# pityka/lamp

Hardware: AMD Instinct MI355X
Metric: training-step samples/sec (higher is better)
Workload: dtype bf16; 1 GPU; example-cifar100 Cnn.resnet(100) training step (fwd+backprop+AdamW), synthetic CIFAR batch; per_gpu_batch=2048, global_batch=2048, parallelism=single, optimizer=AdamW lr 1e-3 wd 0 beta2 0.95 mixedPrecision

## Files before the change

lamp_amd/csrc/core/switches.h:

```cpp
#pragma once
#include <cstdint>

namespace lamp {

constexpr int64_t SW_NO_CLAMP = INT64_MIN;

#define LAMP_SWITCHES_ONCE(X)                                                                                                             \
                                                        \
  X(conv_sibling, "LAMP_CONV_SIBLING", BOOL, 1, 0, "a residual block's 3x3 and its sibling 1x1 of the same input as one forward launch") \
  X(conv_chain, "LAMP_CONV_CHAIN", BOOL, 1, 0, "a convolution directly in front of a residual block and the block's 3x3 + 1x1 as one forward call (0: two)") \
  X(fuse_bn_pair, "LAMP_FUSE_BN_PAIR", BOOL, 1, 0, "relu(bn(right) + bn(left)) at a block's end as one op (0: the chain)")                \
  X(fuse_pool_logsoftmax, "LAMP_FUSE_POOL_LOGSOFTMAX", BOOL, 1, 0, "average pool -> flatten -> log-softmax tail as one node")             \
  X(fuse_block_tail, "LAMP_FUSE_BLOCK_TAIL", BOOL, 1, 0, "the last residual block and the pooled log-softmax tail as one node")          \
  X(fuse_bn_conv, "LAMP_FUSE_BN_CONV", BOOL, 1, 0, "batch norm -> relu -> convolution: the convolution applies the norm while staging")  \
  X(fuse_loss_accumulate, "LAMP_FUSE_LOSS_ACCUMULATE", BOOL, 1, 0, "acc += n * loss inside the NLL loss kernel")                          \
  X(fuse_loss_backward, "LAMP_FUSE_LOSS_BACKWARD", BOOL, 1, 0, "the NLL loss backward goes straight to the pooled log-softmax node's input in one launch")                      \
  X(fuse_loss_tail, "LAMP_FUSE_LOSS_TAIL", BOOL, 1, 0, "the loss launch also writes the pooled log-softmax's input gradient per plane")  \
  X(conv_dgrad_accumulate, "LAMP_CONV_DGRAD_ACCUMULATE", BOOL, 1, 0, "a convolution's input gradient adds into the existing one in its epilogue") \
  X(conv_dgrad_pair, "LAMP_CONV_DGRAD_PAIR", BOOL, 1, 0, "input gradients of a block's 3x3 and sibling 1x1 from one launch")             \
  X(conv_wgrad_pair, "LAMP_CONV_WGRAD_PAIR", BOOL, 1, 0, "weight gradients of a block's 3x3 and sibling 1x1 from one launch")            \
  X(conv_bwd_pair, "LAMP_CONV_BWD_PAIR", BOOL, 1, 0, "a block's paired input gradient and its two weight gradients from one call (0: the two pair calls)") \
  X(linear_bias_fused, "LAMP_LINEAR_BIAS_FUSED", BOOL, 1, 0, "a linear layer's bias in the GEMM epilogue (0: mm then add)")               \
  X(mult_add_fused, "LAMP_MULT_ADD_FUSED", BOOL, 1, 0, "x * scale + residual in one pass (0: mult then add)")                             \
  X(attention_as_written_for_cuda, "LAMP_ATTENTION_AS_WRITTEN_FOR_CUDA", BOOL, 0, 0, "multi-head attention as the reference's op chain instead of the fused kernels") \
  X(recurrent_fused, "LAMP_RECURRENT_FUSED", BOOL, 1, 0, "RNN / GRU / LSTM as one node per sequence with fused cell kernels (0: the fold over time steps)") \
  X(fuse_qkv, "LAMP_FUSE_QKV", BOOL, 1, 0, "self-attention's three projections as one product (0: three)")                                \
  X(host_stream_side, "LAMP_HOST_STREAM_SIDE", BOOL, 0, 0, "batch streams gather on a side stream instead of the consumer's")             \
                                                                           \
  X(pinned_cache_mb, "LAMP_PINNED_CACHE_MB", INT, 2048, 0, "upper bound of the cache of freed pinned host buffers, MiB")                  \
  X(pinned_gather_wgs, "LAMP_PINNED_GATHER_WGS", INT, 48, 1, "workgroups of a gather that reads pinned host memory")                      \
                                                                                                    \
  X(flash_attention, "LAMP_FLASH_ATTENTION", BOOL, 1, 0, "the flash attention kernels, forward and backward")                             \
  X(small_attention, "LAMP_SMALL_ATTENTION", BOOL, 1, 0, "the short-sequence attention kernels")                                          \
  X(knn_fused, "LAMP_KNN_FUSED", BOOL, 1, 0, "the fused distance + top-k nearest-neighbour kernel")                                       \
  X(knn_split, "LAMP_KNN_SPLIT", INT, -1, SW_NO_CLAMP, "f16-plane k-NN filter: 0 off, 1 where it pays, 2 forced; negative: the mode set through the API") \
  X(knn_split_planes, "LAMP_KNN_SPLIT_PLANES", INT, 0, SW_NO_CLAMP, "f16 planes per coordinate of that filter: 3, anything else 2")      \
  X(umap_pairs2, "LAMP_UMAP_PAIRS2", BOOL, 1, 0, "the UMAP loss's two-dimensional pair kernel")                                            \
                                                                                                             \
  X(gemm_shape_tags, "LAMP_GEMM_SHAPE_TAGS", BOOL, 0, 0, "profiling aid: one kernel-timer class per GEMM shape and layout")               \
  X(gemm_splitk, "LAMP_GEMM_SPLITK", BOOL, 1, 0, "split-K for products with few output tiles (bf16 and f32 / f64)")                       \
  X(gemm_tail_split, "LAMP_GEMM_TAIL_SPLIT", BOOL, 1, 0, "an almost empty last round of 256 x 256 tiles becomes a second, split-K product") \
  X(gemm_fp_split_wgs, "LAMP_GEMM_FP_SPLIT_WGS", INT, 512, 1, "workgroups an f32 / f64 split-K product aims at")                          \
                                                                                              \
  X(bn_fused_bwd, "LAMP_BN_FUSED_BWD", BOOL, 1, 0, "one-pass batch-norm backward (workgroups exchange their sums) where no mode is set through the API") \
  X(bn_fused_fp, "LAMP_BN_FUSED_FP", BOOL, 1, 0, "... its f32 / f64 form")                                                               \
  X(bn_fused_np_mask, "LAMP_BN_FUSED_NP_MASK", INT, 24, SW_NO_CLAMP, "bit mask of packets per thread (1 .. 16) at which the one-pass form runs") \
  X(bn_fused_per_cu, "LAMP_BN_FUSED_PER_CU", INT, 1, 1, "workgroups per CU the one-pass form aims at first")                              \
  X(bn_fused_small_bytes, "LAMP_BN_FUSED_SMALL_BYTES", INT, (4 << 20) + 1, SW_NO_CLAMP, "bf16 activations below this many bytes take the one-pass form whatever the mask") \
                          \
  X(conv_small2, "LAMP_CONV_SMALL2", BOOL, 1, 0, "the small-map direct convolution kernels (second generation)")                          \
  X(conv_small2_wgrad, "LAMP_CONV_SMALL2_WGRAD", BOOL, 1, 0, "... their weight gradient")                                                 \
  X(igemm_f32, "LAMP_IGEMM_F32", BOOL, 1, 0, "implicit-GEMM convolution for f32")                                                          \
  X(igemm_f64, "LAMP_IGEMM_F64", BOOL, 1, 0, "implicit-GEMM convolution for f64")                                                          \
  X(conv_bn_stats, "LAMP_CONV_BN_STATS", BOOL, 1, 0, "forward convolutions hand per-image batch-norm statistics of their output on")     \
  X(ncv_bn_stats, "LAMP_NCV_BN_STATS", BOOL, 1, 0, "... the narrow kernels' alone (needs LAMP_CONV_BN_STATS on as well)")                 \
  X(ncv_dgrad_parity, "LAMP_NCV_DGRAD_PARITY", BOOL, 1, 0, "narrow stride-2 pair input gradient: super-tiles by row parity (0: the plain form)") \
  X(pack_cache, "LAMP_PACK_CACHE", BOOL, 1, 0, "packed filter images are cached per parameter and storage version (all four packing backends: core/pack_cache.h)") \
  X(pack_after_step, "LAMP_PACK_AFTER_STEP", BOOL, 1, 0, "the optimiser repacks every cached filter image of all four backends in place (0: lazily at first use)") \
                                                    \
  X(ig_small_d, "LAMP_IG_SMALL_D", BOOL, 1, 0, "the eight-image kernel for at most 64 output channels too")                               \
  X(ig_w8, "LAMP_IG_W8", BOOL, 1, 0, "two-image 128-row kernel: eight waves per image pair at one workgroup per CU or fewer (0: four)")  \
  X(ig_one_image, "LAMP_IG_ONE_IMAGE", BOOL, 1, 0, "... one image per workgroup at one image per CU or fewer (0: pairs)")                 \
  X(ig_bwd_pair, "LAMP_IG_BWD_PAIR", BOOL, 1, 0, "a wide block's short-K entry pair: input gradient and both weight gradients from one eight-image launch (0: the two pair calls)") \
  X(ig_fwd_pair, "LAMP_IG_FWD_PAIR", BOOL, 1, 0, "a wide block's short-K entry pair, forward: the barrier-free eight-image kernel with both filters resident in LDS (0: the eight-image kernel's sibling form)") \
                                                                                                 \
  X(wgrad_group, "LAMP_WGRAD_GROUP", BOOL, 1, 0, "two layers' eight-wave weight gradients parked and launched as one (0: every layer at once)") \
  X(wgrad_min_ips, "LAMP_WGRAD_MIN_IPS", INT, 0, 2, "fewest images per weight-gradient workgroup; unset (0): 2 up to 512 images, 8 above") \
  X(wg8h_dma, "LAMP_WG8H_DMA", BOOL, 1, 0, "eight-wave weight-gradient kernel: dY tiles by LDS-DMA (0: through registers, the bitwise reference of the DMA's hand-counted waits)") \
  X(defer_wgrad_reduce, "LAMP_DEFER_WGRAD_REDUCE", BOOL, 1, 0, "weight-gradient partial sums are reduced in batches, deferred until someone reads them")

#define LAMP_SWITCHES_PER_CALL(X)                                                                                                         \
  X(ig_variant, "LAMP_IG_VARIANT", LETTER, 0, 0, "bf16 implicit GEMM kernel form: b two-image 128-row, d eight-image at any batch; unset or any other letter: by geometry") \
  X(ig_ktail, "LAMP_IG_KTAIL", BOOL, 1, 0, "a 3x3's 1 .. 8 channels beyond the last whole K chunk from their own packed image (0: the padded chunk)") \
  X(knn_split_dbg, "LAMP_KNN_SPLIT_DBG", INT, 0, SW_NO_CLAMP, "3: the k-NN filter's kernel counts visits, candidates and selection cycles per wave and prints them")

using SwType_BOOL = bool;
using SwType_INT = int64_t;
using SwType_LETTER = char;
#define LAMP_SWITCH_MEMBER(member, name, kind, dflt, lo, doc) SwType_##kind member;
struct Switches { LAMP_SWITCHES_ONCE(LAMP_SWITCH_MEMBER) };
struct SwitchesNow { LAMP_SWITCHES_PER_CALL(LAMP_SWITCH_MEMBER) };
#undef LAMP_SWITCH_MEMBER

const Switches& sw();
SwitchesNow sw_now();

}
```

lamp_amd/csrc/host/ops.cpp:

```cpp
#include "ops.h"
#include "../core/switches.h"
#include <cstring>
#include <map>
#include <tuple>

#include <unordered_set>

namespace lamp {
namespace host {

Var make_const(const Ten& t) {
  auto v = std::make_shared<Variable>();
  v->value = t;
  return v;
}
Var make_param(const Ten& t) {
  auto v = std::make_shared<Variable>();
  v->value = t;
  v->wants_grad = true;
  return v;
}
Var make_result(const std::shared_ptr<Op>& op, const Ten& value) {
  auto v = std::make_shared<Variable>();
  v->op = op;
// ... 632 lines not shown
        cache->p = p;
      }
      acc.accumulate(cache->g[which], true);
      cache->g[which] = Ten();
      if (!cache->g[0].defined() && !cache->g[1].defined() && !cache->g[2].defined()) cache->p = Ten();
    };
  };
  op->params.push_back({query, back(0)});
  op->params.push_back({key, back(1)});
  op->params.push_back({value, back(2)});
  return make_result(op, out);
}

struct ConvPairGrad {
  struct Side { Ten w; std::vector<int64_t> stride, padding, dilation; Ten p; Ten pw; Variable* wout = nullptr; };
  Side side[2];
  int64_t groups = 1;
  int waiting = -1;
  int wwaiting = -1;
  Ten dw[2], dwp;
  void drop_merged() { dw[0] = Ten(); dw[1] = Ten(); dwp = Ten(); }
};
static Var convolution_node(const Var& input, const Var& weight, const Var& bias, const std::vector<int64_t>& stride,
                            const std::vector<int64_t>& padding, const std::vector<int64_t>& dilation, bool transposed,
                            const std::vector<int64_t>& outputPadding, int64_t groups, const Ten* computed,
                            const std::shared_ptr<ConvPairGrad>& pair = nullptr, int pair_side = 0) {
  auto op = new_op("Convolution");
  const int ns = (int)stride.size();
  Ten iv = input->value, wv = weight->value;
  const bool fuse_accumulate = sw().conv_dgrad_accumulate;
  const bool fuse_pair = sw().conv_dgrad_pair;
  const bool fuse_bwd_pair = sw().conv_bwd_pair && sw().conv_wgrad_pair;
  Variable* const wvar = weight.get();
  auto back = [=](int which) {
    std::function<void(const Ten&, Variable&)> single;
    single = [=](const Ten& p, Variable& out) {
      if (which == 0 && !transposed && fuse_accumulate && out.has_grad() && out.grad.h()->is_device() && p.h()->is_device() && out.grad.dtype() == p.dtype()) {
        lamp_tensor* r = nullptr;
        HCALL(lamp_convolution_backward_input_add(&r, p.h(), iv.h(), wv.h(), stride.data(), padding.data(), dilation.data(), ns,
                                                  outputPadding.data(), groups, out.grad.h()));
        out.grad = Ten(r);
        out.grad_shared = false;
        return;
      }
      lamp_tensor* o3[3] = {nullptr, nullptr, nullptr};
      uint8_t mask[3] = {(uint8_t)(which == 0), (uint8_t)(which == 1), (uint8_t)(which == 2)};
      HCALL(lamp_convolution_backward(o3, p.h(), iv.h(), wv.h(), stride.data(), padding.data(), dilation.data(), ns, transposed,
                                      outputPadding.data(), groups, mask));
      out.accumulate(Ten(o3[which]), true);
    };
    const bool fuse_wpair = sw().conv_wgrad_pair;
    if (which == 1 && pair && fuse_wpair && !transposed) {
      Variable* inp = input.get();
      return Backward([=](const Ten& p, Variable& out) {
        if (!p.h()->is_device() || tls_backprop_hooked || out.op) { single(p, out); return; }
        ConvPairGrad& st = *pair;
        if (st.wwaiting < 0) {
          st.wwaiting = pair_side;
          st.side[pair_side].pw = p;
          st.side[pair_side].wout = &out;
          inp->pending.push_back([=] {
            ConvPairGrad& s2 = *pair;
            if (s2.wwaiting != pair_side) return;
            s2.drop_merged();
            const Ten held = s2.side[pair_side].pw;
            Variable* wo = s2.side[pair_side].wout;
            s2.side[pair_side].pw = Ten(); s2.side[pair_side].wout = nullptr; s2.wwaiting = -1;
            single(held, *wo);
          });
          return;
        }
        if (st.wwaiting == pair_side) { single(p, out); return; }
        const int other = st.wwaiting;
        const Ten po = st.side[other].pw;
        Variable* wo = st.side[other].wout;
        st.side[other].pw = Ten(); st.side[other].wout = nullptr; st.wwaiting = -1;
        if (st.dw[0].defined() && st.dwp.defined() && st.dwp.h() == p.h()) {
          const Ten da = st.dw[0], db = st.dw[1];
          st.drop_merged();
          (pair_side == 0 ? out : *wo).accumulate(da, true);
          (pair_side == 0 ? *wo : out).accumulate(db, true);
// ... 28 lines not shown
        });
        return;
      }
      if (st.waiting == pair_side) { single(p, out); return; }
      const int other = st.waiting;
      const Ten po = st.side[other].p;
      st.side[other].p = Ten(); st.waiting = -1;
      const Ten& pa = pair_side == 0 ? p : po;
      const Ten& pb = pair_side == 0 ? po : p;
      const bool have = out.has_grad() && out.grad.h()->is_device() && out.grad.dtype() == p.dtype();
      if (out.has_grad() && !have) { single(po, out); single(p, out); return; }
      if (fuse_bwd_pair && !tls_backprop_hooked && st.wwaiting == other && st.side[other].pw.defined() && st.side[other].pw.h() == po.h() &&
          st.side[other].wout && !wvar->op && wvar->needsGrad() && wvar->value.h()->is_device()) {
        lamp_tensor* o3[3] = {nullptr, nullptr, nullptr};
        HCALL(lamp_convolution_backward_pair(o3, iv.h(), pa.h(), st.side[0].w.h(), st.side[0].stride.data(), st.side[0].padding.data(),
                                             st.side[0].dilation.data(), pb.h(), st.side[1].w.h(), st.side[1].stride.data(),
                                             st.side[1].padding.data(), st.side[1].dilation.data(), ns, st.groups, have ? out.grad.h() : nullptr));
        out.grad = Ten(o3[0]);
        out.grad_shared = false;
        st.dw[0] = Ten(o3[1]); st.dw[1] = Ten(o3[2]); st.dwp = p;
        return;
      }
      lamp_tensor* r = nullptr;
      HCALL(lamp_convolution_backward_input_pair(&r, iv.h(), pa.h(), st.side[0].w.h(), st.side[0].stride.data(), st.side[0].padding.data(),
                                                 st.side[0].dilation.data(), pb.h(), st.side[1].w.h(), st.side[1].stride.data(),
                                                 st.side[1].padding.data(), st.side[1].dilation.data(), ns, st.groups, have ? out.grad.h() : nullptr));
      out.grad = Ten(r);
      out.grad_shared = false;
    });
  };
  op->params.push_back({input, back(0)});
  op->params.push_back({weight, back(1)});
  op->params.push_back({bias, back(2)});
  if (pair) op->reset = [pair] {
    pair->waiting = pair->wwaiting = -1;
    for (auto& sd : pair->side) { sd.p = Ten(); sd.pw = Ten(); sd.wout = nullptr; }
    pair->drop_merged();
  };
  if (computed) return make_result(op, *computed);
  lamp_tensor* o = nullptr;
  HCALL(lamp_convolution(&o, iv.h(), wv.h(), bias->value.h(), stride.data(), padding.data(), dilation.data(), ns, transposed,
                         outputPadding.data(), groups));
  return make_result(op, Ten(o));
}
Var convolution(const Var& input, const Var& weight, const Var& bias, const std::vector<int64_t>& stride,
                const std::vector<int64_t>& padding, const std::vector<int64_t>& dilation, bool transposed,
                const std::vector<int64_t>& outputPadding, int64_t groups) {
  return convolution_node(input, weight, bias, stride, padding, dilation, transposed, outputPadding, groups, nullptr);
}
static std::pair<Var, Var> convolution_pair_nodes(const Var& input, const Var& weight_a, const Var& bias_a, const std::vector<int64_t>& stride_a,
                                                  const std::vector<int64_t>& padding_a, const std::vector<int64_t>& dilation_a, const Var& weight_b,
                                                  const Var& bias_b, const std::vector<int64_t>& stride_b, const std::vector<int64_t>& padding_b,
                                                  const std::vector<int64_t>& dilation_b, int64_t groups, const Ten& ya, const Ten& yb);
std::pair<Var, Var> convolution_pair(const Var& input, const Var& weight_a, const Var& bias_a, const std::vector<int64_t>& stride_a,
                                     const std::vector<int64_t>& padding_a, const std::vector<int64_t>& dilation_a, const Var& weight_b,
                                     const Var& bias_b, const std::vector<int64_t>& stride_b, const std::vector<int64_t>& padding_b,
                                     const std::vector<int64_t>& dilation_b, int64_t groups) {
  const int ns = (int)stride_a.size();
  LAMP_CHECK(ns == (int)stride_b.size(), "convolution_pair: the two convolutions have different numbers of spatial dimensions");
  lamp_tensor* o2[2] = {nullptr, nullptr};
  HCALL(lamp_convolution_pair(o2, input->value.h(), weight_a->value.h(), bias_a->value.h(), stride_a.data(), padding_a.data(), dilation_a.data(),
                              weight_b->value.h(), bias_b->value.h(), stride_b.data(), padding_b.data(), dilation_b.data(), ns, groups));
  return convolution_pair_nodes(input, weight_a, bias_a, stride_a, padding_a, dilation_a, weight_b, bias_b, stride_b, padding_b, dilation_b, groups, Ten(o2[0]),
                                Ten(o2[1]));
}
static std::pair<Var, Var> convolution_pair_nodes(const Var& input, const Var& weight_a, const Var& bias_a, const std::vector<int64_t>& stride_a,
// ... 419 lines not shown
```

lamp_amd/csrc/kernels/conv.hip:

```cpp
#include "device_utils.h"
#include "../core/strided.h"
#include "../core/switches.h"
#include "conv_geom.h"
#include "conv_backends.h"

namespace lamp {

template <class T>
__global__ __launch_bounds__(256) void conv_fwd_direct_kernel(const T* __restrict__ x, const T* __restrict__ w, const T* __restrict__ bias,
                                                              T* __restrict__ y, ConvGeom g) {
  using A = acc_t<T>;
  const int64_t total = g.N * g.Cout * g.Ho * g.Wo;
  const int cin_g = (int)(g.Cin / g.groups), cout_g = (int)(g.Cout / g.groups);
  for (int64_t e = blockIdx.x * (int64_t)blockDim.x + threadIdx.x; e < total; e += (int64_t)gridDim.x * blockDim.x) {
    const int wo = (int)(e % g.Wo);
    const int ho = (int)((e / g.Wo) % g.Ho);
    const int co = (int)((e / (g.Wo * g.Ho)) % g.Cout);
    const int64_t n = e / (g.Wo * g.Ho * g.Cout);
    const int grp = co / cout_g;
    A acc = bias ? load_as<A>(bias[co]) : A(0);
    const T* wp = w + (int64_t)co * cin_g * g.kh * g.kw;
    for (int cl = 0; cl < cin_g; cl++) {
      const T* xp = x + ((n * g.Cin + grp * cin_g + cl) * g.H) * g.W;
      for (int r = 0; r < g.kh; r++) {
// ... 373 lines not shown
      }
    }
  }
  if (!fused) {
    lamp_tensor* s = nullptr;
    if (lamp_convolution(&s, x, w, bias, stride, padding, dilation, nspatial, 0, zero2, groups) != 0) throw Error(lamp_last_error());
    Hold hs(s);
    lamp_tensor* o2[2] = {nullptr, nullptr};
    if (lamp_convolution_pair(o2, s, w_a, bias_a, stride_a, padding_a, dilation_a, w_b, bias_b, stride_b, padding_b, dilation_b, nspatial, groups) != 0)
      throw Error(lamp_last_error());
    out3[0] = hs.take(); out3[1] = o2[0]; out3[2] = o2[1];
  }
  LAMP_API_END
}

int lamp_convolution_backward(lamp_tensor* out3[3], const lamp_tensor* grad_out, const lamp_tensor* x, const lamp_tensor* w,
                              const int64_t* stride, const int64_t* padding, const int64_t* dilation, int nspatial, int transposed,
                              const int64_t* output_padding, int64_t groups, const uint8_t mask[3]) {
  LAMP_API_BEGIN
  check_device_tensor(x, "input"); check_device_tensor(w, "weight"); check_device_tensor(grad_out, "grad_out");
  LAMP_CHECK(x->dtype == w->dtype && grad_out->dtype == x->dtype, "convolution_backward: dtype mismatch");
  ConvGeom g = make_geom(x, w, stride, padding, dilation, nspatial, transposed, output_padding, groups);
  {
    const int64_t oc = transposed ? g.Cin : g.Cout, oh = transposed ? g.H : g.Ho, ow = transposed ? g.W : g.Wo;
    LAMP_CHECK(grad_out->ndim == x->ndim && grad_out->sizes[0] == g.N && grad_out->sizes[1] == oc &&
               grad_out->sizes[grad_out->ndim - 1] == ow && (nspatial == 1 || grad_out->sizes[2] == oh),
               "convolution_backward: grad_out " << grad_out->describe() << " does not match the forward output shape");
  }
  Hold xc(contiguous(x)), wc(contiguous_filter(w)), gc(contiguous(grad_out));
  hipStream_t st = current_stream(x->device());
  Hold dx(mask[0] ? new_like(xc.get()) : nullptr);
  Hold dw(mask[1] ? new_like(wc.get()) : nullptr);
  Hold db;
  if (!transposed) {
    if (dx.get() && !igemm_conv_dgrad(gc.get(), wc.get(), dx.get(), g, st) && !igemm32_conv_dgrad(gc.get(), wc.get(), dx.get(), g, st) &&
        !narrow_conv_dgrad(gc.get(), wc.get(), dx.get(), g, st) && !small_conv_dgrad(gc.get(), wc.get(), dx.get(), g, st)) {
      LAMP_DISPATCH_FLOAT(x->dtype, T, (launch_dgrad<T>(gc.get(), wc.get(), nullptr, dx.get(), g, st)));
    }
    if (dw.get() && !igemm_conv_wgrad(gc.get(), xc.get(), dw.get(), g, st) && !igemm32_conv_wgrad(gc.get(), xc.get(), dw.get(), g, st) &&
        !narrow_conv_wgrad(gc.get(), xc.get(), dw.get(), g, st) && !small_conv_wgrad(gc.get(), xc.get(), dw.get(), g, st)) {
      LAMP_DISPATCH_FLOAT(x->dtype, T, (launch_wgrad<T>(gc.get(), xc.get(), dw.get(), g, st)));
    }
  } else {
    if (dx.get()) { LAMP_DISPATCH_FLOAT(x->dtype, T, (launch_fwd<T>(gc.get(), wc.get(), nullptr, dx.get(), g, st))); }
    if (dw.get()) { LAMP_DISPATCH_FLOAT(x->dtype, T, (launch_wgrad<T>(xc.get(), gc.get(), dw.get(), g, st))); }
  }
  if (mask[2]) {
    std::vector<int64_t> dims = {0};
    for (int i = 2; i < grad_out->ndim; i++) dims.push_back(i);
    db = Hold(reduce_dims(gc.get(), dims.data(), (int)dims.size(), false, 0));
  }
  out3[0] = dx.take(); out3[1] = dw.take(); out3[2] = db.take();
  LAMP_API_END
}

static void check_affine(const lamp_tensor* affine, const lamp_tensor* x) {
  check_device_tensor(affine, "affine");
  LAMP_CHECK(affine->dtype == kF32 && affine->ndim == 2 && affine->sizes[0] == x->sizes[1] && affine->sizes[1] == 4 && affine->is_contiguous(),
             "affine must be the contiguous f32 [channels, 4] table of lamp_batch_norm_affine, got " << affine->describe());
  LAMP_CHECK(x->dtype == kBF16 || x->dtype == kF16 || x->dtype == kF32, "conv(relu(bn(x))) with a folded batch norm is a reduced-precision path (f32 table): f64 runs the separate operators");
}
int lamp_convolution_bn_relu_input_folds(int* out, const lamp_tensor* x, const lamp_tensor* w, const int64_t* stride, const int64_t* padding,
                                         const int64_t* dilation, int nspatial, int64_t groups) {
  LAMP_API_BEGIN
  *out = 0;
  if (!x->is_device() || !w->is_device() || x->dtype != w->dtype) return 0;
  const int64_t zero2[2] = {0, 0};
// ... 220 lines not shown
```

lamp_amd/csrc/kernels/conv_backends.h:

```cpp
#pragma once
#include "../core/tensor.h"
#include "conv_geom.h"

namespace lamp {
struct NcvPackMany;

bool igemm_conv_fwd(const Tensor* x, const Tensor* w, const Tensor* bias, Tensor* y, const ConvGeom& g, hipStream_t st);
bool igemm_conv_fwd_pair(const Tensor* x, const Tensor* w, const Tensor* bias, Tensor* y, const ConvGeom& g, const Tensor* w1, const Tensor* bias1,
                         Tensor* y1, const ConvGeom& g1, hipStream_t st);
bool igemm_conv_dgrad(const Tensor* dy, const Tensor* w, Tensor* dx, const ConvGeom& g, hipStream_t st, const Tensor* addend = nullptr,
                      bool* addend_fused = nullptr);
bool igemm_conv_dgrad_pair(const Tensor* dy, const Tensor* w, const ConvGeom& g, const Tensor* dy1, const Tensor* w1, const ConvGeom& g1, Tensor* dx,
                           hipStream_t st, const Tensor* addend, bool* addend_fused);
bool igemm_conv_wgrad(const Tensor* dy, const Tensor* x, Tensor* dw, const ConvGeom& g, hipStream_t st, const Tensor* affine = nullptr);
bool igemm_conv_wgrad_pair(const Tensor* dy, const Tensor* dy1, const Tensor* x, Tensor* dw, Tensor* dw1, const ConvGeom& g, const ConvGeom& g1, hipStream_t st);
bool igemm_conv_backward_pair(const Tensor* dy, const Tensor* dy1, const Tensor* x, const Tensor* w, const Tensor* w1, const ConvGeom& g, const ConvGeom& g1,
                              Tensor* dx, Tensor* dw, Tensor* dw1, hipStream_t st, const Tensor* addend = nullptr);
bool igemm_conv_folds_affine(const ConvGeom& g, int dtype);
bool igemm_conv_fwd_affine(const Tensor* x, const Tensor* affine, const Tensor* w, const Tensor* bias, Tensor* y, const ConvGeom& g, hipStream_t st);

bool igemm32_conv_fwd(const Tensor* x, const Tensor* w, const Tensor* bias, Tensor* y, const ConvGeom& g, hipStream_t st);
bool igemm32_conv_dgrad(const Tensor* dy, const Tensor* w, Tensor* dx, const ConvGeom& g, hipStream_t st, const Tensor* addend = nullptr,
                        bool* addend_fused = nullptr);
bool igemm32_conv_wgrad(const Tensor* dy, const Tensor* x, Tensor* dw, const ConvGeom& g, hipStream_t st);

bool narrow_conv_fwd(const Tensor* x, const Tensor* w, const Tensor* bias, Tensor* y, const ConvGeom& g, hipStream_t st);
bool narrow_conv_fwd_pair(const Tensor* x, const Tensor* w, const Tensor* bias, Tensor* y, const ConvGeom& g, const Tensor* w1, const Tensor* bias1,
                          Tensor* y1, const ConvGeom& g1, hipStream_t st);
bool narrow_conv_chain_pair(const Tensor* x, const Tensor* w0, const Tensor* bias0, Tensor* s, const ConvGeom& g0, const Tensor* w, const Tensor* bias,
                            Tensor* y, const ConvGeom& g, const Tensor* w1, const Tensor* bias1, Tensor* y1, const ConvGeom& g1, hipStream_t st);
bool narrow_conv_dgrad(const Tensor* dy, const Tensor* w, Tensor* dx, const ConvGeom& g, hipStream_t st, const Tensor* addend = nullptr,
                       bool* addend_fused = nullptr);
bool narrow_conv_dgrad_pair(const Tensor* dy, const Tensor* w, const ConvGeom& g, const Tensor* dy1, const Tensor* w1, const ConvGeom& g1, Tensor* dx,
                            hipStream_t st, const Tensor* addend, bool* addend_fused);
bool narrow_conv_wgrad(const Tensor* dy, const Tensor* x, Tensor* dw, const ConvGeom& g, hipStream_t st);
bool narrow_conv_backward_pair(const Tensor* dy, const Tensor* dy1, const Tensor* x, const Tensor* w, const Tensor* w1, const ConvGeom& g, const ConvGeom& g1,
                               Tensor* dx, Tensor* dw, Tensor* dw1, hipStream_t st, const Tensor* addend = nullptr);
bool narrow_conv_wgrad_pair(const Tensor* dy, const Tensor* dy1, const Tensor* x, Tensor* dw, Tensor* dw1, const ConvGeom& g, const ConvGeom& g1, hipStream_t st);

bool small_conv_fwd(const Tensor* x, const Tensor* w, const Tensor* bias, Tensor* y, const ConvGeom& g, hipStream_t st);
bool small_conv_dgrad(const Tensor* dy, const Tensor* w, Tensor* dx, const ConvGeom& g, hipStream_t st, const Tensor* addend = nullptr,
                      bool* addend_fused = nullptr);
bool small_conv_wgrad(const Tensor* dy, const Tensor* x, Tensor* dw, const ConvGeom& g, hipStream_t st);

void conv_repack_cached(lamp_tensor* const* params, int n, hipStream_t st);
void igemm_repack_cached(lamp_tensor* const* params, int n, hipStream_t st);
void igemm32_repack_cached(lamp_tensor* const* params, int n, hipStream_t st);
void small_repack_cached(lamp_tensor* const* params, int n, hipStream_t st);
void narrow_repack_cached(lamp_tensor* const* params, int n, hipStream_t st, NcvPackMany* fill, int* fill_cnt);
void narrow_pack_launch(const NcvPackMany& a, int cnt, hipStream_t st);

}
```

lamp_amd/csrc/kernels/conv_narrow.hip:

```cpp
#include "device_utils.h"
#include "conv_geom.h"
#include "conv_backends.h"
#include "../core/pack_cache.h"
#include "wgrad_reduce.h"
#include <type_traits>
#include <vector>
#include "conv_narrow_pack.h"
#include "../core/switches.h"

namespace lamp {

typedef nv_s8 __attribute__((aligned(2))) nv_s8_u;
typedef float nv_f4 __attribute__((ext_vector_type(4)));

struct NcvGeom {
  int N, C, CO;
  int H, W;
  int Hs, Ws;
  int top, left, dil;
  int Ho, Wo;
  int sh, sw, wx;
  int kh;
  int kh_inv;
  int pf;
// ... 594 lines not shown
        const int b = e % rcd, a = (e / rcd) % q.Ho, c = e / (rcd * q.Ho) + (second ? qd.C1 : 0);
        pl.dst2[k] = (c * qd.Hs + qd.top + a * qd.dil) * qd.Ws + qd.left + b * 8 * qd.dil;
      }
    }
  }
  return pf;
}
template <int WPF>
__device__ __forceinline__ void ncv_wg_load(uint4 (&pre)[WPF], const NcvWPlan<WPF>& pl, const NcvWGeom& q, const bf16_t* __restrict__ x, const bf16_t* __restrict__ dy,
                                            const bf16_t* __restrict__ dy2, int64_t nb, int ig) {
  const int HoWo = q.Ho * q.Wo;
  const bf16_t* xg = x + nb * q.Cin * q.H * q.W;
  const bf16_t* dg = dy + nb * q.Cout * HoWo;
  const bf16_t* dg2 = dy2 + nb * q.Cout2 * HoWo;
#pragma unroll
  for (int k = 0; k < WPF; k++)
    if (pl.im[k] >= 0 && pl.im[k] < ig) {
      const bf16_t* sp = pl.src[k] >= 0 ? xg + pl.src[k] : pl.src[k] >= -(1 << 30) ? dg + (-pl.src[k] - 1) : dg2 + (-pl.src[k] - 1 - (1 << 30));
      pre[k] = *reinterpret_cast<const uint4*>(sp);
    }
}
template <int SW>
__device__ __forceinline__ void ncv_wg_stage_x(unsigned short* dst, const uint4 v, int Ws) {
  if (SW == 1) {
    *reinterpret_cast<uint4*>(dst) = v;
  } else {
    uint2 ev, od;
    ev.x = (v.x & 0xffffu) | (v.y << 16); ev.y = (v.z & 0xffffu) | (v.w << 16);
    od.x = (v.x >> 16) | (v.y & 0xffff0000u); od.y = (v.z >> 16) | (v.w & 0xffff0000u);
    *reinterpret_cast<uint2*>(dst) = ev;
    *reinterpret_cast<uint2*>(dst + Ws) = od;
  }
}
template <int SW, int WPF, bool DIL>
__device__ __forceinline__ void ncv_wg_store(unsigned short* xs, unsigned short* xd, const uint4 (&pre)[WPF], const NcvWPlan<WPF>& pl, int ig, int Ws, int dil) {
#pragma unroll
  for (int k = 0; k < WPF; k++) {
    if (pl.im[k] < 0 || pl.im[k] >= ig) continue;
    const uint4 v = pre[k];
    if (SW == 1 || pl.src[k] < 0) *reinterpret_cast<uint4*>(xs + pl.dst[k]) = v;
    else ncv_wg_stage_x<SW>(xs + pl.dst[k], v, Ws);
    if (DIL && pl.dst2[k] >= 0) ncv_scatter8(xd + pl.dst2[k], v, dil);
  }
}
template <int SW, int NPT>
__device__ __forceinline__ void ncv_wg_pair_offsets(const NcvWGeom& q, int lane, int (&poff)[NPT]) {
  const int npairs = q.Cin * q.kh;
#pragma unroll
  for (int pt = 0; pt < NPT; pt++) {
    int pair = pt * 16 + (lane & 15);
    if (pair >= npairs) pair = 0;
    const int ci = pair / q.kh, r = pair - ci * q.kh;
    poff[pt] = (SW == 1 ? (ci * q.Hs + r) * q.Ws : (ci * q.Hs + r) * 2 * q.Ws) * 2;
  }
}
template <int KW, int PW, int SW, int NPT, bool W2>
__device__ __forceinline__ void ncv_wg_chunks(const unsigned short* xs, const unsigned short* ds, int drows, const NcvWGeom& q, int ximg, const int (&poff)[NPT],
                                              nv_f4 (&acc)[NPT][KW], nv_f4 (&acc2)[NPT], int nchunks, int wid, int lane) {
  const int HoWo = q.Ho * q.Wo;
  for (int ch = wid; ch < nchunks; ch += 4) {
    const int pg = ch * 32 + (lane >> 4) * 8;
    const int im = pg / HoWo, pp = pg - im * HoWo;
    const int ho = pp / q.Wo, wo0 = pp - ho * q.Wo;
    const nv_s8 a = *reinterpret_cast<const nv_s8*>(ds + (im * drows + (lane & 15)) * HoWo + pp);
    const nv_bf8 af = __builtin_bit_cast(nv_bf8, a);
    nv_bf8 af2 = af;
    if constexpr (W2) af2 = __builtin_bit_cast(nv_bf8, *reinterpret_cast<const nv_s8*>(ds + (im * drows + 16 + (lane & 15)) * HoWo + pp));
    const char* xb = reinterpret_cast<const char*>(xs + im * ximg) +
                     (SW == 1 ? (ho * q.Ws + wo0 + NCV_OFFA - 8) * 2 : ((ho * 2) * 2 * q.Ws + wo0 + NCV_OFFA - 8) * 2);
#pragma unroll
    for (int pt = 0; pt < NPT; pt++) {
      const char* rowp = xb + poff[pt];
      if (SW == 1) {
        constexpr bool need_m = PW > 0, need_p = (KW - 1 - PW) > 0;
        unsigned int sg[13];
// ... 188 lines not shown
  }
  const int co = lane & 7;
  const int ncg = qd.Wo / 8;
  const int a_tr = (lane & 15) / ncg, a_cg = (lane & 15) - a_tr * ncg;
  const int a_off = (2 * a_tr * qd.sh * qd.Ws + a_cg * 8 + (qd.wx - PH0)) * 2;
  const int HoWo_d = qd.Ho * qd.Wo;
  NcvStatAcc none{nv_f4{0.f, 0.f, 0.f, 0.f}, nv_f4{0.f, 0.f, 0.f, 0.f}, 0};
  const int chunks_per_img = HoWo >> 5;
  for (int64_t nb = n0; nb < n1; nb += q.IG) {
    const int ig = (int)min<int64_t>(q.IG, n1 - nb);
    __syncthreads();
    ncv_wg_store<SW, WPF, true>(xs, xd, pre, plan, ig, q.Ws, qd.dil);
    __syncthreads();
    if (nb + q.IG < n1) ncv_wg_load(pre, plan, q, x, dy, dy2, nb + q.IG, (int)min<int64_t>(q.IG, n1 - nb - q.IG));
    ncv_wg_chunks<KW, PW, SW, NPT, W2>(xs, ds, drows, q, ximg, poff, acc, acc2, ig * chunks_per_img, wid, lane);
    for (int im = 0; im < ig; im++) {
      if (im > 0) {
        __syncthreads();
        const NcvPlanT<2> dplan = ncv_stage_plan<2>(qd, tid, 256);
        const bf16_t* pa = reinterpret_cast<const bf16_t*>(ds + im * drows * HoWo);
        NcvPreT<2> t;
        ncv_stage_load(t, dplan, pa, pa + (W2 ? 16 : q.Cout) * HoWo);
        ncv_stage_store(xd, t, dplan, qd.dil);
        __syncthreads();
      }
      const int64_t n = nb + im;
      bf16_t* yc = dx + (n * qd.CO + co) * HoWo_d;
      const bf16_t* ap = ADD ? add + (n * qd.CO + co) * HoWo_d : nullptr;
      ncv_super_tiles<NK, 1, PH0, NS, ADD, false, true, false, NK / 2, (NK >= 8 ? 2 : 0)>(reinterpret_cast<const char*>(xd), qd, wfr, koff, a_off, 0.f, co, yc, ap, none, nullptr, 0, lane, wid, 4);
    }
  }
  __syncthreads();
  ncv_wg_finish<KW, NPT, W2>(red, red2, acc, acc2, q, partial, partial2, tid, 256, wid, lane);
}


static inline int round_up(int v, int m) { return (v + m - 1) / m * m; }

static bool ncv_common(const ConvGeom& g, int dtype) {
  if (dtype != kBF16) return false;
  if (g.groups != 1 || g.transposed || g.dh != 1 || g.dw != 1) return false;
  if (g.Cin > 16 || g.Cout > 16 || g.N < 1) return false;
  if (g.sh != g.sw || g.sh < 1 || g.sh > 2) return false;
  if (g.kw > 8 || g.ph > g.kh - 1 || g.pw > g.kw - 1 || g.pw > 8) return false;
  return true;
}

static bool ncv_pair_shapes(const ConvGeom& g, const ConvGeom& g1) {
  if (g.kh != 3 || g.kw != 3 || g.ph != 1 || g.pw != 1 || g1.kh != 1 || g1.kw != 1 || g1.ph != 0 || g1.pw != 0) return false;
  if (g.sh != g1.sh || g.sw != g1.sw || g.Ho != g1.Ho || g.Wo != g1.Wo || g.H != g1.H || g.W != g1.W || g.Cin != g1.Cin || g.N != g1.N) return false;
  return g.groups == 1 && g1.groups == 1 && g.dh == 1 && g.dw == 1 && g1.dh == 1 && g1.dw == 1;
}
static double ncv_sibling_flops(const ConvGeom& g, int cout2) { return 2.0 * (double)g.N * cout2 * (double)g.Ho * g.Wo * (double)g.Cin; }
static double ncv_sibling_bytes(const ConvGeom& g, int cout2) { return ((double)g.N * cout2 * g.Ho * g.Wo + (double)cout2 * g.Cin) * 2.0; }

constexpr size_t NCV_LDS_BUDGET = 150 * 1024;
constexpr size_t NCV_LDS_DEFAULT = 64 * 1024;
constexpr int NCV_PER_CU_MAX = 4;
static int ncv_lds_per_cu(size_t lds) { return (int)std::max<size_t>(1, std::min<size_t>(NCV_PER_CU_MAX, NCV_LDS_BUDGET / std::max<size_t>(lds, 1))); }
static int ncv_per_cu(const void* kfn, int threads, size_t lds) { return std::min(ncv_lds_per_cu(lds), kernel_occupancy(kfn, threads, lds)); }
static void ncv_launch(const void* kfn, int blocks, int threads, size_t lds, void** args, hipStream_t st) {
  if (lds > NCV_LDS_DEFAULT) allow_big_lds(kfn);
  HIP_CHECK(hipLaunchKernel(kfn, dim3(blocks), dim3(threads), args, lds, st));
  LAMP_LAUNCH_CHECK();
}
struct NcvStats {
// ... 466 lines not shown
  if (q.IG * per > NCV_WPF * 256) return false;
  const int threads = 256;
  if (q.IG > 1 && (int64_t)qd.C * qd.H * qd.W > (int64_t)2 * threads * 8) return false;
  const bool with_add = addend != nullptr;
  const void* kfn = nullptr;
#define NCV_BP(NKv, W2v, WPFv) kfn = with_add ? (const void*)ncv_bwd_pair_kernel<NKv, true, 2, W2v, WPFv> : (const void*)ncv_bwd_pair_kernel<NKv, false, 2, W2v, WPFv>
  if (lp.NK == 6 && !w2) NCV_BP(6, false, NCV_WPF);
  else if (lp.NK == 8 && !w2) NCV_BP(8, false, NCV_WPF);
  else if (lp.NK == 16 && q.IG * per <= 4 * 256) { if (w2) NCV_BP(16, true, 4); else NCV_BP(16, false, 4); }
  else return false;
#undef NCV_BP
  const int per_cu = std::min(ncv_per_cu(ref.kfn, 256, ref.lds), ncv_per_cu(kfn, threads, lds));
  int ipb = 0;
  const int nblocks = ncv_partition(per_cu, g.N, ref.q.IG, ipb);
  Hold wpk_h(ncv_packed_weights(w, ncv_weights_of(w, g, true, lp, w1, cout2), st, w1));
  const nv_bf8* wpk = ncv_fragments(wpk_h);
  const int O = q.Cout * q.ncol, O2 = cout2 * q.Cin;
  Hold partial(new_tensor({(int64_t)nblocks * O}, kF32, dy->device())), partial2(new_tensor({(int64_t)nblocks * O2}, kF32, dy->device()));
  {
    const double dy_by = (double)g.N * (g.Cout + cout2) * HoWo * 2.0;
    KernelTimer kt("conv_bwd_narrow", 2.0 * (conv_flops(g) + ncv_sibling_flops(g, cout2)), 2.0 * (conv_bytes(g, 2) + ncv_sibling_bytes(g, cout2)) - dy_by, st);
    const bf16_t* dp = dy->ptr<bf16_t>(); const bf16_t* dp2 = dy1->ptr<bf16_t>(); const bf16_t* xp = x->ptr<bf16_t>();
    bf16_t* dxp = dx->ptr<bf16_t>();
    const bf16_t* addp = with_add ? addend->ptr<bf16_t>() : (const bf16_t*)nullptr;
    float* pp = partial->ptr<float>(); float* pp2 = partial2->ptr<float>();
    void* args[] = {(void*)&dp, (void*)&dp2, (void*)&xp, (void*)&wpk, (void*)&dxp, (void*)&addp, (void*)&pp, (void*)&pp2, (void*)&q, (void*)&qd, (void*)&ipb};
    ncv_launch(kfn, nblocks, threads, lds, args, st);
  }
  wgrad_reduce_flat(O, nblocks, partial.get(), dw, st);
  wgrad_reduce_flat(O2, nblocks, partial2.get(), dw1, st);
  return true;
}

}
```

Baseline: 2.330 million samples/s.

## Fuse narrow 3x3 conv input and weight gradients into one backward launch

Adds a kernel that computes a narrow stride-1 3x3 convolution's input gradient and weight-gradient partial sums in a single pass, sharing the staged dy tiles in LDS. On the host, the input-gradient callback also requests the weight gradient and parks it, and the weight callback then picks up the parked result instead of launching separately. This avoids reading dy and x twice and saves one launch per block. In exchange the kernel needs more LDS and may run at lower occupancy, and the host-side parking adds state that must be reset between steps.

```diff
diff --git a/lamp_amd/csrc/core/switches.h b/lamp_amd/csrc/core/switches.h
--- a/lamp_amd/csrc/core/switches.h
+++ b/lamp_amd/csrc/core/switches.h
@@ -55,6 +55,7 @@
   X(conv_bn_stats, "LAMP_CONV_BN_STATS", BOOL, 1, 0, "forward convolutions hand per-image batch-norm statistics of their output on")     \
   X(ncv_bn_stats, "LAMP_NCV_BN_STATS", BOOL, 1, 0, "... the narrow kernels' alone (needs LAMP_CONV_BN_STATS on as well)")                 \
   X(ncv_dgrad_parity, "LAMP_NCV_DGRAD_PARITY", BOOL, 1, 0, "narrow stride-2 pair input gradient: super-tiles by row parity (0: the plain form)") \
+  X(ncv_bwd_single, "LAMP_NCV_BWD_SINGLE", BOOL, 1, 0, "a narrow block's second 3x3: input gradient and weight gradient from one launch (0: the two launches)") \
   X(pack_cache, "LAMP_PACK_CACHE", BOOL, 1, 0, "packed filter images are cached per parameter and storage version (all four packing backends: core/pack_cache.h)") \
   X(pack_after_step, "LAMP_PACK_AFTER_STEP", BOOL, 1, 0, "the optimiser repacks every cached filter image of all four backends in place (0: lazily at first use)") \
                                                     \
diff --git a/lamp_amd/csrc/host/ops.cpp b/lamp_amd/csrc/host/ops.cpp
--- a/lamp_amd/csrc/host/ops.cpp
+++ b/lamp_amd/csrc/host/ops.cpp
@@ -688,9 +688,17 @@
   const bool fuse_pair = sw().conv_dgrad_pair;
   const bool fuse_bwd_pair = sw().conv_bwd_pair && sw().conv_wgrad_pair;
   Variable* const wvar = weight.get();
+  struct Merged { Ten dw, dwp; void drop() { dw = Ten(); dwp = Ten(); } };
+  const std::shared_ptr<Merged> mg = (!pair && !transposed && sw().ncv_bwd_single) ? std::make_shared<Merged>() : nullptr;
   auto back = [=](int which) {
     std::function<void(const Ten&, Variable&)> single;
     single = [=](const Ten& p, Variable& out) {
+      if (which == 1 && mg && mg->dw.defined()) {
+        const Ten dw = mg->dw;
+        const bool mine = mg->dwp.h() == p.h();
+        mg->drop();
+        if (mine) { out.accumulate(dw, true); return; }
+      }
       if (which == 0 && !transposed && fuse_accumulate && out.has_grad() && out.grad.h()->is_device() && p.h()->is_device() && out.grad.dtype() == p.dtype()) {
         lamp_tensor* r = nullptr;
         HCALL(lamp_convolution_backward_input_add(&r, p.h(), iv.h(), wv.h(), stride.data(), padding.data(), dilation.data(), ns,
@@ -701,8 +709,11 @@
       }
       lamp_tensor* o3[3] = {nullptr, nullptr, nullptr};
       uint8_t mask[3] = {(uint8_t)(which == 0), (uint8_t)(which == 1), (uint8_t)(which == 2)};
+      const bool both = which == 0 && mg && p.h()->is_device() && !tls_backprop_hooked && !wvar->op && wvar->needsGrad() && wvar->value.h()->is_device();
+      if (both) mask[1] = 1;
       HCALL(lamp_convolution_backward(o3, p.h(), iv.h(), wv.h(), stride.data(), padding.data(), dilation.data(), ns, transposed,
                                       outputPadding.data(), groups, mask));
+      if (both) { mg->dw = Ten(o3[1]); mg->dwp = p; }
       out.accumulate(Ten(o3[which]), true);
     };
     const bool fuse_wpair = sw().conv_wgrad_pair;
@@ -797,6 +808,7 @@
   op->params.push_back({input, back(0)});
   op->params.push_back({weight, back(1)});
   op->params.push_back({bias, back(2)});
+  if (mg) op->reset = [mg] { mg->drop(); };
   if (pair) op->reset = [pair] {
     pair->waiting = pair->wwaiting = -1;
     for (auto& sd : pair->side) { sd.p = Ten(); sd.pw = Ten(); sd.wout = nullptr; }
diff --git a/lamp_amd/csrc/kernels/conv.hip b/lamp_amd/csrc/kernels/conv.hip
--- a/lamp_amd/csrc/kernels/conv.hip
+++ b/lamp_amd/csrc/kernels/conv.hip
@@ -429,7 +429,10 @@
   Hold dx(mask[0] ? new_like(xc.get()) : nullptr);
   Hold dw(mask[1] ? new_like(wc.get()) : nullptr);
   Hold db;
-  if (!transposed) {
+  const bool merged = !transposed && mask[0] && mask[1] && !mask[2] && nspatial == 2 &&
+                      narrow_conv_backward_single(gc.get(), xc.get(), wc.get(), g, dx.get(), dw.get(), st);
+  if (merged) {
+  } else if (!transposed) {
     if (dx.get() && !igemm_conv_dgrad(gc.get(), wc.get(), dx.get(), g, st) && !igemm32_conv_dgrad(gc.get(), wc.get(), dx.get(), g, st) &&
         !narrow_conv_dgrad(gc.get(), wc.get(), dx.get(), g, st) && !small_conv_dgrad(gc.get(), wc.get(), dx.get(), g, st)) {
       LAMP_DISPATCH_FLOAT(x->dtype, T, (launch_dgrad<T>(gc.get(), wc.get(), nullptr, dx.get(), g, st)));
diff --git a/lamp_amd/csrc/kernels/conv_backends.h b/lamp_amd/csrc/kernels/conv_backends.h
--- a/lamp_amd/csrc/kernels/conv_backends.h
+++ b/lamp_amd/csrc/kernels/conv_backends.h
@@ -36,6 +36,7 @@
 bool narrow_conv_wgrad(const Tensor* dy, const Tensor* x, Tensor* dw, const ConvGeom& g, hipStream_t st);
 bool narrow_conv_backward_pair(const Tensor* dy, const Tensor* dy1, const Tensor* x, const Tensor* w, const Tensor* w1, const ConvGeom& g, const ConvGeom& g1,
                                Tensor* dx, Tensor* dw, Tensor* dw1, hipStream_t st, const Tensor* addend = nullptr);
+bool narrow_conv_backward_single(const Tensor* dy, const Tensor* x, const Tensor* w, const ConvGeom& g, Tensor* dx, Tensor* dw, hipStream_t st);
 bool narrow_conv_wgrad_pair(const Tensor* dy, const Tensor* dy1, const Tensor* x, Tensor* dw, Tensor* dw1, const ConvGeom& g, const ConvGeom& g1, hipStream_t st);
 
 bool small_conv_fwd(const Tensor* x, const Tensor* w, const Tensor* bias, Tensor* y, const ConvGeom& g, hipStream_t st);
diff --git a/lamp_amd/csrc/kernels/conv_narrow.hip b/lamp_amd/csrc/kernels/conv_narrow.hip
--- a/lamp_amd/csrc/kernels/conv_narrow.hip
+++ b/lamp_amd/csrc/kernels/conv_narrow.hip
@@ -650,7 +650,7 @@
     *reinterpret_cast<uint2*>(dst + Ws) = od;
   }
 }
-template <int SW, int WPF, bool DIL>
+template <int SW, int WPF, bool DIL, bool PACKET = false>
 __device__ __forceinline__ void ncv_wg_store(unsigned short* xs, unsigned short* xd, const uint4 (&pre)[WPF], const NcvWPlan<WPF>& pl, int ig, int Ws, int dil) {
 #pragma unroll
   for (int k = 0; k < WPF; k++) {
@@ -658,7 +658,8 @@
     const uint4 v = pre[k];
     if (SW == 1 || pl.src[k] < 0) *reinterpret_cast<uint4*>(xs + pl.dst[k]) = v;
     else ncv_wg_stage_x<SW>(xs + pl.dst[k], v, Ws);
-    if (DIL && pl.dst2[k] >= 0) ncv_scatter8(xd + pl.dst2[k], v, dil);
+    if constexpr (PACKET) { if (DIL && pl.dst2[k] >= 0) *reinterpret_cast<uint4*>(xd + pl.dst2[k]) = v; }
+    else if (DIL && pl.dst2[k] >= 0) ncv_scatter8(xd + pl.dst2[k], v, dil);
   }
 }
 template <int SW, int NPT>
@@ -913,6 +914,57 @@
   }
   __syncthreads();
   ncv_wg_finish<KW, NPT, W2>(red, red2, acc, acc2, q, partial, partial2, tid, 256, wid, lane);
+}
+
+template <int NK, int NS, int NPT, int WPF>
+__global__ __launch_bounds__(256, NPT <= 2 ? 3 : 2) void ncv_bwd_single_kernel(const bf16_t* __restrict__ dy, const bf16_t* __restrict__ x, const nv_bf8* __restrict__ wpk,
+                                                                                  bf16_t* dx, float* __restrict__ partial, NcvWGeom q, NcvGeom qd, int images_per_block) {
+  constexpr int KW = 3, PW = 1, SW = 1, PH0 = 7;
+  extern __shared__ __attribute__((aligned(16))) char smem[];
+  const int tid = threadIdx.x, lane = tid & 63, wid = tid >> 6;
+  const int HoWo = q.Ho * q.Wo;
+  const int ximg = q.Cin * q.Hs * q.Ws;
+  unsigned short* xs = reinterpret_cast<unsigned short*>(smem);
+  unsigned short* ds = xs + ximg;
+  unsigned short* xd = ds + 16 * HoWo;
+  float* red = reinterpret_cast<float*>(xd);
+  const int64_t n0 = (int64_t)blockIdx.x * images_per_block, n1 = min<int64_t>(n0 + images_per_block, q.N);
+  uint4 pre[WPF];
+  NcvWPlan<WPF> plan;
+  ncv_wg_plan<SW, WPF, true>(plan, q, ximg, 16, q.Cout, tid, 256, qd);
+  if (n0 < n1) ncv_wg_load(pre, plan, q, x, dy, dy, n0, 1);
+  nv_bf8 wfr[NK];
+  int koff[NK];
+  ncv_frag_setup<NK, false>(qd, wpk, lane, wfr, koff);
+  {
+    const int tot = ximg + 16 * HoWo + qd.C * qd.Hs * qd.Ws;
+    for (int o = tid * 8; o < tot; o += 256 * 8) *reinterpret_cast<uint4*>(xs + o) = make_uint4(0, 0, 0, 0);
+  }
+  int poff[NPT];
+  ncv_wg_pair_offsets<SW, NPT>(q, lane, poff);
+  nv_f4 acc[NPT][KW], none2[NPT];
+#pragma unroll
+  for (int pt = 0; pt < NPT; pt++)
+#pragma unroll
+    for (int s = 0; s < KW; s++) acc[pt][s] = nv_f4{0.f, 0.f, 0.f, 0.f};
+  const int co = NS == 2 ? (lane & 7) : (lane & 15);
+  const int ncg = qd.Wo / 8;
+  const int a_tr = (lane & 15) / ncg, a_cg = (lane & 15) - a_tr * ncg;
+  const int a_off = (a_tr * qd.sh * qd.Ws + a_cg * 8 + (qd.wx - PH0)) * 2;
+  const int HoWo_d = qd.Ho * qd.Wo;
+  NcvStatAcc none{nv_f4{0.f, 0.f, 0.f, 0.f}, nv_f4{0.f, 0.f, 0.f, 0.f}, 0};
+  const int chunks_per_img = HoWo >> 5;
+  for (int64_t n = n0; n < n1; n++) {
+    __syncthreads();
+    ncv_wg_store<SW, WPF, true, true>(xs, xd, pre, plan, 1, q.Ws, 1);
+    __syncthreads();
+    if (n + 1 < n1) ncv_wg_load(pre, plan, q, x, dy, dy, n + 1, 1);
+    ncv_wg_chunks<KW, PW, SW, NPT, false>(xs, ds, 16, q, ximg, poff, acc, none2, chunks_per_img, wid, lane);
+    ncv_super_tiles<NK, 1, PH0, NS, false, false, false, false, NK, (NK >= 8 ? 2 : 0)>(reinterpret_cast<const char*>(xd), qd, wfr, koff, a_off, 0.f, co,
+                                                                                        dx + (n * qd.CO + co) * HoWo_d, nullptr, none, nullptr, 0, lane, wid, 4);
+  }
+  __syncthreads();
+  ncv_wg_finish<KW, NPT, false>(red, nullptr, acc, none2, q, partial, nullptr, tid, 256, wid, lane);
 }
 
 
@@ -1445,4 +1497,44 @@
   return true;
 }
 
-}
+constexpr int64_t NCV_BWD_SINGLE_MIN_N = 64;
+bool narrow_conv_backward_single(const Tensor* dy, const Tensor* x, const Tensor* w, const ConvGeom& g, Tensor* dx, Tensor* dw, hipStream_t st) {
+  if (!sw().ncv_bwd_single) return false;
+  if (x->dtype != kBF16 || dy->dtype != kBF16 || w->dtype != kBF16) return false;
+  if (g.kh != 3 || g.kw != 3 || g.ph != 1 || g.pw != 1 || g.sh != 1 || g.sw != 1 || g.N < NCV_BWD_SINGLE_MIN_N) return false;
+  NcvLaunchPlan lp;
+  if (!ncv_plan(g, x->dtype, true, false, false, 0, true, lp)) return false;
+  if (!lp.aligned || lp.nke != 0 || lp.ph0 != 7 || lp.q.sw != 1 || lp.q.dil != 1 || lp.q.W % 8 != 0 || !(lp.NK == 5 || lp.NK == 12)) return false;
+  const NcvGeom& qd = lp.q;
+  NcvWgradPlan ref;
+  if (!ncv_wgrad_plan(g, x->dtype, 0, true, ref) || ref.q.IG != 1) return false;
+  const NcvWGeom& q = ref.q;
+  const int HoWo = q.Ho * q.Wo, ximg = q.Cin * q.Hs * q.Ws;
+  const size_t red_bytes = (size_t)4 * 16 * ref.npt * 3 * 16 * 4;
+  const size_t lds = (size_t)(ximg + 16 * HoWo) * 2 + std::max(lp.lds, red_bytes);
+  if (lds > NCV_LDS_BUDGET) return false;
+  const int per = (q.Cin * q.H * q.W + q.Cout * HoWo) >> 3;
+  const void* kfn = nullptr;
+  if (lp.NS == 2 && ref.npt == 2 && lp.NK == 5 && per <= 2 * 256) kfn = (const void*)ncv_bwd_single_kernel<5, 2, 2, 2>;
+  else if (lp.NS == 1 && ref.npt == 3 && lp.NK == 5 && per <= 4 * 256) kfn = (const void*)ncv_bwd_single_kernel<5, 1, 3, 4>;
+  else if (lp.NS == 1 && ref.npt == 3 && lp.NK == 12 && per <= 4 * 256) kfn = (const void*)ncv_bwd_single_kernel<12, 1, 3, 4>;
+  if (!kfn) return false;
+  if (ncv_per_cu(ref.kfn, 256, ref.lds) > (ref.npt <= 2 ? 3 : 2)) return false;
+  Hold wpk_h(ncv_packed_weights(w, ncv_weights_of(w, g, true, lp, nullptr, 0), st));
+  const nv_bf8* wpk = ncv_fragments(wpk_h);
+  const int O = q.Cout * q.ncol;
+  Hold partial(new_tensor({(int64_t)ref.nblocks * O}, kF32, dy->device()));
+  {
+    KernelTimer kt("conv_dgrad_narrow", 2.0 * conv_flops(g), 2.0 * conv_bytes(g, 2) - (double)g.N * g.Cout * HoWo * 2.0, st);
+    const bf16_t* dp = dy->ptr<bf16_t>(); const bf16_t* xp = x->ptr<bf16_t>();
+    bf16_t* dxp = dx->ptr<bf16_t>();
+    float* pp = partial->ptr<float>();
+    int ipb = ref.ipb;
+    void* args[] = {(void*)&dp, (void*)&xp, (void*)&wpk, (void*)&dxp, (void*)&pp, (void*)&q, (void*)&qd, (void*)&ipb};
+    ncv_launch(kfn, ref.nblocks, 256, lds, args, st);
+  }
+  wgrad_reduce_flat(O, ref.nblocks, partial.get(), dw, st);
+  return true;
+}
+
+}
```

Measured after the change: 2.346 million samples/s (median of 6 runs). No clear change (+0.7%).
